# XMUDM/SPEX

Hardware: NVIDIA B200
Metric: lightgcn_propagation_gedges_per_s (higher is better)
Workload: dtype f32

## Files before the change

### include/spex_b200.h

```cpp
#ifndef SPEX_B200_H
#define SPEX_B200_H

#include <stdint.h>

#ifdef __cplusplus
extern "C" {
#endif

#define SPEX_ABI_VERSION 1

#define SPEX_E_BADARG   (-1)
#define SPEX_E_BADDIM   (-2)
#define SPEX_E_ALIGN    (-3)
#define SPEX_E_ARCH     (-4)
#define SPEX_E_TOOBIG   (-5)
#define SPEX_E_WORKSPACE (-6)

int spex_abi_version(void);
const char* spex_error_string(int code);
int spex_device_check(int* sm_count, int* cc_major, int* cc_minor);
int64_t spex_launch_count(void);

#define SPEX_PLAN_COL_HOTBIT 1
#define SPEX_PLAN_TWO_PASS 2
#define SPEX_PLAN_INTERLEAVE 4

typedef struct spex_long_plan {
  int32_t seg_len;
  int32_t n_long;
  int32_t n_seg;
  int32_t flags;
  const int32_t* long_rows;
  const int32_t* long_segptr;
  float* partial;
  const int64_t* seg_start;
  const int32_t* seg_count;
  const int32_t* row_seg;
  const int64_t* rowmid;
  float* hot_partial;
  int64_t n_split_rows;
  int64_t interleave_split;
} spex_long_plan;

int spex_spmm_csr_f32(const int64_t* rowptr, const int32_t* col, const float* val,
                      const float* X, int64_t n_rows, int32_t D,
                      float* Y, const float* addend, float addend_scale,
                      float* Z, float z_scale,
                      const spex_long_plan* plan, void* stream);

int spex_spmm_csr_rows_f32(const int64_t* rowptr, const int32_t* col, const float* val,
                           const float* X, int64_t n_rows, int32_t D,
                           const int32_t* rows, int64_t n_sel,
                           const int32_t* long_slots, int32_t n_long_sel,
                           const int32_t* seg_ids, int32_t n_seg_sel,
                           const uint8_t* x_nonzero,
                           float* Y, const float* addend, float addend_scale,
                           float* Z, float z_scale,
                           const spex_long_plan* plan, void* stream);

int spex_propagate_mean_f32(const int64_t* rowptr, const int32_t* col, const float* val,
                            const float* E0, int64_t N, int32_t D, int32_t K,
                            float* out, float* tmp0, float* tmp1,
                            const spex_long_plan* plan, void* stream);

int spex_propagate_mean_bwd_f32(const int64_t* rowptr, const int32_t* col, const float* valT,
                                const float* g, int64_t N, int32_t D, int32_t K,
                                float* dE0, float* tmp0, float* tmp1,
                                const spex_long_plan* plan, void* stream);

int spex_gather_f32(const float* src, const int64_t* idx, const float* scale, float divisor,
                    float* out, int64_t n, void* stream);

int spex_bce_fwd_f32(const float* U, const float* I, int32_t D,
                     const int64_t* users, const int64_t* items, const float* labels,
                     int64_t B, float* gamma, float* loss, float* dgamma, void* stream);

int spex_bce_bwd_f32(const float* U, const float* I, int32_t D,
                     const int64_t* users, const int64_t* items, const float* dgamma,
                     const float* grad_loss, int64_t B, float* gU, float* gI, void* stream);
int64_t spex_scatter_workspace_bytes(int64_t total_entries);
int spex_bce_bwd_ws_f32(const float* U, const float* I, int32_t D,
                        const int64_t* users, const int64_t* items, const float* dgamma,
                        const float* grad_loss, int64_t B, float* gU, float* gI,
                        void* work, int64_t work_bytes, void* stream);
int spex_clear_rows_f32(float* table, const int64_t* rows, int64_t n, int32_t D, void* stream);
int spex_gather_owned_rows_f32(const float* table_local, const int64_t* rows, int64_t n, int32_t D,
                               int64_t row_lo, int64_t row_hi, float* R, void* stream);
int spex_scatter_rows_f32(const int64_t* dst_rows, const int64_t* src_rows, const float* coef,
                          const float* gscalar, float cconst, int64_t B, const float* src, int32_t D,
                          float* out, int64_t row_lo, int64_t row_hi, void* work, int64_t work_bytes,
                          void* stream);

int spex_bpr_fwd_f32(const float* U, const float* I, const float* U0, const float* I0, int32_t D,
                     const int64_t* users, const int64_t* pos, const int64_t* neg, int64_t B,
// ... 126 lines not shown
```

### spex_b200/_capi.py

```python
from __future__ import annotations

import ctypes as C
import os

_HERE = os.path.dirname(os.path.abspath(__file__))
LIB_PATH = os.environ.get("SPEX_B200_LIB") or os.path.join(_HERE, "libspex_b200.so")

_p = C.c_void_p
_i32 = C.c_int32
_i64 = C.c_int64
_f = C.c_float


class LongPlan(C.Structure):

    _fields_ = [
        ("seg_len", _i32),
        ("n_long", _i32),
        ("n_seg", _i32),
        ("flags", _i32),
        ("long_rows", _p),
        ("long_segptr", _p),
        ("partial", _p),
        ("seg_start", _p),
        ("seg_count", _p),
        ("row_seg", _p),
        ("rowmid", _p),
        ("hot_partial", _p),
        ("n_split_rows", _i64),
        ("interleave_split", _i64),
    ]


_PLAN = C.POINTER(LongPlan)

SIGNATURES = {
    "spex_abi_version": (C.c_int, []),
    "spex_error_string": (C.c_char_p, [C.c_int]),
    "spex_device_check": (C.c_int, [C.POINTER(C.c_int)] * 3),
    "spex_launch_count": (_i64, []),
    "spex_spmm_csr_f32": (C.c_int, [_p, _p, _p, _p, _i64, _i32, _p, _p, _f, _p, _f, _PLAN, _p]),
    "spex_spmm_csr_rows_f32": (C.c_int, [_p, _p, _p, _p, _i64, _i32, _p, _i64, _p, _i32, _p, _i32, _p, _p, _p, _f, _p, _f,
                                         _PLAN, _p]),
    "spex_spmm_csr_rows_exchange_f32": (C.c_int, [_p, _p, _p, _p, _i64, _i32, _p, _i64, _p, _i32, _p, _i32, _p, _i64, _p,
                                                  _p, _i32, _p, _f, _p, _f, _PLAN, _p]),
    "spex_propagate_mean_f32": (C.c_int, [_p, _p, _p, _p, _i64, _i32, _i32, _p, _p, _p, _PLAN, _p]),
    "spex_propagate_mean_bwd_f32": (C.c_int, [_p, _p, _p, _p, _i64, _i32, _i32, _p, _p, _p, _PLAN, _p]),
    "spex_gather_f32": (C.c_int, [_p, _p, _p, _f, _p, _i64, _p]),
    "spex_bce_fwd_f32": (C.c_int, [_p, _p, _i32, _p, _p, _p, _i64, _p, _p, _p, _p]),
    "spex_bce_bwd_f32": (C.c_int, [_p, _p, _i32, _p, _p, _p, _p, _i64, _p, _p, _p]),
    "spex_scatter_workspace_bytes": (_i64, [_i64]),
    "spex_bce_bwd_ws_f32": (C.c_int, [_p, _p, _i32, _p, _p, _p, _p, _i64, _p, _p, _p, _i64, _p]),
    "spex_clear_rows_f32": (C.c_int, [_p, _p, _i64, _i32, _p]),
    "spex_gather_owned_rows_f32": (C.c_int, [_p, _p, _i64, _i32, _i64, _i64, _p, _p]),
    "spex_scatter_rows_f32": (C.c_int, [_p, _p, _p, _p, _f, _i64, _p, _i32, _p, _i64, _i64, _p, _i64, _p]),
    "spex_bpr_bwd_ws_f32": (C.c_int, [_p, _p, _p, _p, _i32, _p, _p, _p, _p, _p, _i64, _p, _p, _p, _p, _p, _i64, _p]),
    "spex_bpr_fwd_f32": (C.c_int, [_p, _p, _p, _p, _i32, _p, _p, _p, _i64, _p, _p, _p, _p]),
    "spex_bpr_bwd_f32": (C.c_int, [_p, _p, _p, _p, _i32, _p, _p, _p, _p, _p, _i64, _p, _p, _p, _p, _p]),
    "spex_adam_f32": (C.c_int, [_p, _p, _p, _p, _i64, _f, _f, _f, _f, _i32, _p]),
    "spex_sample_negatives": (C.c_int, [_p, _p, _i32, _i32, _p, _i64, _i32, C.c_uint64, _p, _p]),
    "spex_sample_bpr": (C.c_int, [_p, _p, _i32, _i32, _i64, _i64, C.c_uint64, _p, _p, _p, _p]),
    "spex_expert_gate_f32": (C.c_int, [_p, _p, _p, _i64, _i32, _p, _p]),
    "spex_expert_gate_bwd_f32": (C.c_int, [_p, _p, _p, _p, _i64, _i32, _p, _p, _p, _p, _p]),
    "spex_score_topk_f32": (C.c_int, [_p, _p, _i32, _p, _i64, _i64, _p, _p, _i32, _p, _p, _p]),
    "spex_rating_f32": (C.c_int, [_p, _p, _i32, _p, _i64, _i64, _i32, _p, _p]),
    "spex_pack_bf16": (C.c_int, [_p, _p, _i64, _i64, _i32, _p, _p]),
    "spex_score_topk_bf16": (C.c_int, [_p, _p, _i64, _i64, _i64, _i64, _p, _p, _p, _i32, _p, _p, _p]),
    "spex_pack_f16": (C.c_int, [_p, _p, _i64, _i64, _i32, _p, _p, _p]),
    "spex_score_topk_f16": (C.c_int, [_p, _p, _i32, _i64, _i64, _i64, _i64, _p, _p, _p, _p, _p, _i32, _p, _p, _p]),
    "spex_score_candidates_f32": (C.c_int, [_p, _p, _i32, _p, _p, _i64, _i32, _p, _p]),
    "spex_ngcf_epilogue_f32": (C.c_int, [_p, _p, _p, _p, _p, _p, _i64, _i32, _f, _p, _p, _i64, _p]),
    "spex_ngcf_layer_fwd_f32": (C.c_int, [_p, _p, _p, _p, _p, _p, _p, _i64, _i32, _f, _p, _p, _i64, _p]),
    "spex_ngcf_layer_bwd_f32": (C.c_int, [_p, _p, _p, _p, _p, _p, _p, _p, _p, _i64, _i64, _i32, _f, _p, _p, _p, _p,
                                          _p, _p, _p, _p]),
    "spex_ipc_alloc": (C.c_int, [_i64, C.POINTER(_p), _p]),
    "spex_ipc_open": (C.c_int, [_p, C.POINTER(_p)]),
    "spex_ipc_close": (C.c_int, [_p]),
    "spex_ipc_free": (C.c_int, [_p]),
    "spex_spmm_csr_f32_mcast": (C.c_int, [_p, _p, _p, _p, _i64, _i32, _i64, _p, _p, _f, _p, _f, _PLAN, _p]),
    "spex_mcast_rows_f32": (C.c_int, [_p, _i64, _i32, _i64, _p, _p]),
    "spex_mcast_rows_f32_ex": (C.c_int, [_p, _i64, _i32, _i64, _p, _i32, _p]),
    "spex_push_rows_f32_ex": (C.c_int, [_p, _i64, _i32, _i64, C.POINTER(_p), _i32, _i32, _p]),
    "spex_spmm_csr_f32_publish": (C.c_int, [_p, _p, _p, _p, _i64, _i32, _i64, _p, _f, _p, _f, _p, _p,
# ... 79 lines not shown
```

### spex_b200/csrc/spmm.cu

```cuda
#include "common.cuh"
#include <math.h>
#include <stdlib.h>

namespace spex {

int64_t g_launches = 0;

template <int D>
struct RowShape {
  static_assert(D == 32 || D == 64 || D == 128, "vector path supports D in {32,64,128}");
  static constexpr int LPR = D / 4;
  static constexpr int G = 32 / LPR;
};

template <int D, int U, int kMode, bool kFirst = false, bool kHot = false>
__device__ __forceinline__ float4 warp_row_accumulate(const int32_t* __restrict__ col,
                                                      const float* __restrict__ val,
                                                      const float* __restrict__ X, int64_t start,
                                                      int64_t end, int lane, int c0 = 0,
                                                      float v0 = 0.f) {
  constexpr int LPR = RowShape<D>::LPR, G = RowShape<D>::G;
  const int grp = lane / LPR, sub = lane % LPR;
  const float* Xs = X + sub * 4;
  float4 acc = f4_zero();
// ... 24 lines not shown
    const int n = (int)((end - base) < 32 ? (end - base) : 32);
#pragma unroll 1
    for (int j = 0; j < n; j += G * U) {
      float4 x[U];
      float vv[U];
#pragma unroll
      for (int u = 0; u < U; ++u) {
        const int idx = j + u * G + grp;
        const int cc = __shfl_sync(kFull, c, idx & 31);
        vv[u] = __shfl_sync(kFull, v, idx & 31);
        if (idx < n) {
          if (kHot)
            x[u] = ld_gather_f4_hint(Xs + (int64_t)(cc & 0x7fffffff) * D, cc < 0 ? pol_last : pol_first);
          else
            x[u] = ld_gather_f4(Xs + (int64_t)cc * D);
        } else {
          x[u] = f4_zero();
          vv[u] = 0.f;
        }
      }
#pragma unroll
      for (int u = 0; u < U; ++u) f4_fma(acc, vv[u], x[u]);
    }
  }
#pragma unroll
  for (int m = LPR; m < 32; m <<= 1) f4_add(acc, f4_shfl_xor(acc, m));
  return acc;
}

struct f8 {
  float4 a, b;
};
__device__ __forceinline__ f8 ld_gather_f8(const float* p) {
  f8 v;
  asm("ld.global.nc.L1::no_allocate.v8.f32 {%0,%1,%2,%3,%4,%5,%6,%7}, [%8];"
      : "=f"(v.a.x), "=f"(v.a.y), "=f"(v.a.z), "=f"(v.a.w), "=f"(v.b.x), "=f"(v.b.y), "=f"(v.b.z), "=f"(v.b.w)
      : "l"(p));
  return v;
}
__device__ __forceinline__ f8 ld_gather_f8_last(const float* p) {
  f8 v;
  asm("ld.global.nc.L1::no_allocate.L2::evict_last.v8.f32 {%0,%1,%2,%3,%4,%5,%6,%7}, [%8];"
      : "=f"(v.a.x), "=f"(v.a.y), "=f"(v.a.z), "=f"(v.a.w), "=f"(v.b.x), "=f"(v.b.y), "=f"(v.b.z), "=f"(v.b.w)
      : "l"(p));
  return v;
}
__device__ __forceinline__ f8 ld_gather_f8_first(const float* p) {
  f8 v;
  asm("ld.global.nc.L1::no_allocate.L2::evict_first.v8.f32 {%0,%1,%2,%3,%4,%5,%6,%7}, [%8];"
      : "=f"(v.a.x), "=f"(v.a.y), "=f"(v.a.z), "=f"(v.a.w), "=f"(v.b.x), "=f"(v.b.y), "=f"(v.b.z), "=f"(v.b.w)
      : "l"(p));
  return v;
}
template <int D, bool kHot>
__device__ __forceinline__ f8 gather_row8(const float* Xs, int cc) {
  const float* p;
  asm("mad.wide.u32 %0, %1, %2, %3;" : "=l"(p) : "r"(kHot ? (uint32_t)cc & 0x7fffffffu : (uint32_t)cc), "n"(D * 4), "l"(Xs));
  if (kHot) return cc < 0 ? ld_gather_f8_last(p) : ld_gather_f8_first(p);
  return ld_gather_f8(p);
}
__device__ __forceinline__ void f8_fma(f8& acc, float s, const f8& x) {
  f4_fma(acc.a, s, x.a);
  f4_fma(acc.b, s, x.b);
}

template <int D, int U, bool kHot>
__device__ __forceinline__ float4 warp_row_accumulate8(const int32_t* __restrict__ col,
                                                       const float* __restrict__ val,
                                                       const float* __restrict__ X, int64_t start,
                                                       int64_t end, int lane) {
  constexpr int LPR8 = D / 8;
  static_assert(LPR8 % U == 0, "U must divide the group's share of a batch");
  const int grp = lane / LPR8, sub = lane % LPR8;
  const float* Xs = X + sub * 8;
  f8 acc;
  acc.a = f4_zero();
  acc.b = f4_zero();
  int rem = (int)(end - start);
  const int32_t* cp = col + start + lane;
  const float* vp = val + start + lane;
  int c = 0;
  float v = 0.f;
  if (lane < rem) {
    c = ld_stream_s32(cp);
    v = ld_stream_f32(vp);
  }
  while (rem > 0) {
    int cn = 0;
    float vn = 0.f;
    if (lane + 32 < rem) {
      cn = ld_stream_s32(cp + 32);
      vn = ld_stream_f32(vp + 32);
    }
    if (rem >= 32) {
#pragma unroll
      for (int k0 = 0; k0 < LPR8; k0 += U) {
        f8 x[U];
        float vv[U];
#pragma unroll
        for (int u = 0; u < U; ++u) {
          const int cc = __shfl_sync(kFull, c, k0 + u, LPR8);
          vv[u] = __shfl_sync(kFull, v, k0 + u, LPR8);
          x[u] = gather_row8<D, kHot>(Xs, cc);
        }
#pragma unroll
        for (int u = 0; u < U; ++u) f8_fma(acc, vv[u], x[u]);
      }
    } else {
      const int ng = rem - grp * LPR8;
      const int nmax = rem < LPR8 ? rem : LPR8;
#pragma unroll 1
      for (int k0 = 0; k0 < nmax; k0 += U) {
        f8 x[U];
        float vv[U];
#pragma unroll
        for (int u = 0; u < U; ++u) {
          const int cc = __shfl_sync(kFull, c, k0 + u, LPR8);
          vv[u] = __shfl_sync(kFull, v, k0 + u, LPR8);
          if (k0 + u < ng) {
            x[u] = gather_row8<D, kHot>(Xs, cc);
          } else {
            x[u].a = f4_zero();
            x[u].b = f4_zero();
            vv[u] = 0.f;
          }
        }
#pragma unroll
        for (int u = 0; u < U; ++u) f8_fma(acc, vv[u], x[u]);
      }
    }
    c = cn;
    v = vn;
    cp += 32;
    vp += 32;
    rem -= 32;
  }
#pragma unroll
  for (int m = LPR8; m < 32; m <<= 1) {
    f4_add(acc.a, f4_shfl_xor(acc.a, m));
    f4_add(acc.b, f4_shfl_xor(acc.b, m));
  }
  const int src = (lane >> 1) & (LPR8 - 1);
  float4 lo, hi;
  lo.x = __shfl_sync(kFull, acc.a.x, src);
  lo.y = __shfl_sync(kFull, acc.a.y, src);
  lo.z = __shfl_sync(kFull, acc.a.z, src);
  lo.w = __shfl_sync(kFull, acc.a.w, src);
  hi.x = __shfl_sync(kFull, acc.b.x, src);
  hi.y = __shfl_sync(kFull, acc.b.y, src);
  hi.z = __shfl_sync(kFull, acc.b.z, src);
  hi.w = __shfl_sync(kFull, acc.b.w, src);
  return (lane & 1) ? hi : lo;
}

#ifndef SPEX_V8_U
#define SPEX_V8_U 4
#endif
#ifndef SPEX_MASK_U
#define SPEX_MASK_U 2
#endif
#ifndef SPEX_V8_MINB
#define SPEX_V8_MINB 32
#endif
template <int D, bool kHot>
__device__ __forceinline__ float4 warp_row_accumulate8_masked(const int32_t* __restrict__ col,
                                                              const float* __restrict__ val,
                                                              const float* __restrict__ X,
                                                              const uint8_t* __restrict__ nz, int64_t start,
                                                              int64_t end, int lane) {
  constexpr int LPR8 = D / 8;
  constexpr int U = SPEX_MASK_U;
  const int grp = lane / LPR8, sub = lane % LPR8;
  const float* Xs = X + sub * 8;
  f8 acc;
  acc.a = f4_zero();
  acc.b = f4_zero();
  int rem = (int)(end - start);
  const int32_t* cp = col + start + lane;
  const float* vp = val + start + lane;
  constexpr uint32_t kIdMask = kHot ? 0x7fffffffu : 0xffffffffu;
  int c = 0, cn = 0;
  float v = 0.f, vn = 0.f;
  bool on = false;
  if (lane < rem) {
    c = ld_stream_s32(cp);
    v = ld_stream_f32(vp);
  }
  if (lane + 32 < rem) {
    cn = ld_stream_s32(cp + 32);
    vn = ld_stream_f32(vp + 32);
  }
  if (lane < rem) on = nz[(uint32_t)c & kIdMask] != 0;
  while (rem > 0) {
    int c2 = 0;
// ... 185 lines not shown
                     const int32_t* __restrict__ long_rows,
                     const int32_t* __restrict__ long_segptr, int32_t n_long, int32_t n_seg,
                     int32_t seg_len, float* __restrict__ partial, const int32_t* __restrict__ seg_sel,
                     const uint8_t* __restrict__ nz) {
  constexpr int LPR = RowShape<D>::LPR;
  const int lane = threadIdx.x & 31;
  int seg = blockIdx.x * kRowsPerCta + (threadIdx.x >> 5);
  if (seg >= n_seg) return;
  if (seg_sel) seg = seg_sel[seg];
  int lo = 0, hi = n_long;
  while (hi - lo > 1) {
    const int mid = (lo + hi) >> 1;
    if (long_segptr[mid] <= seg) lo = mid; else hi = mid;
  }
  const int64_t row = long_rows[lo];
  const int k = seg - long_segptr[lo];
  const int64_t rs = rowptr[row], re = rowptr[row + 1];
  const int64_t start = rs + (int64_t)k * seg_len;
  const int64_t end = (start + seg_len < re) ? start + seg_len : re;
  const float4 acc = row_sum<D, U, kHot, kV8, kMask>(col, val, X, start, end, lane, nz);
  if (lane < LPR) *reinterpret_cast<float4*>(partial + (int64_t)seg * D + lane * 4) = acc;
}

template <int D, int U>
__global__ void __launch_bounds__(kRowsPerCta * 32)
spmm_long_fix_kernel(const int32_t* __restrict__ long_rows,
                     const int32_t* __restrict__ long_segptr, int32_t n_long,
                     const float* __restrict__ partial, Epilogue ep, const int32_t* __restrict__ slot_sel) {
  const int lane = threadIdx.x & 31;
  int r = blockIdx.x * kRowsPerCta + (threadIdx.x >> 5);
  if (r >= n_long) return;
  if (slot_sel) r = slot_sel[r];
  const float4 acc = warp_row_accumulate<D, U, 1>(nullptr, nullptr, partial, long_segptr[r],
                                                  long_segptr[r + 1], lane);
  row_epilogue<D>(ep, acc, (int64_t)long_rows[r], lane);
}

template <int D, int U, bool kHot, bool kV8, bool kMask>
__global__ void __launch_bounds__(kRowsPerCta * 32, SPEX_V8_MINB / kRowsPerCta)
spmm_seg_list_kernel(const int32_t* __restrict__ col, const float* __restrict__ val,
                     const float* __restrict__ X, const int64_t* __restrict__ seg_start,
                     const int32_t* __restrict__ seg_count, int32_t n_seg, float* __restrict__ partial,
                     const int32_t* __restrict__ seg_sel, const uint8_t* __restrict__ nz) {
  constexpr int LPR = RowShape<D>::LPR;
  const int lane = threadIdx.x & 31;
  int seg = blockIdx.x * kRowsPerCta + (threadIdx.x >> 5);
  if (seg >= n_seg) return;
  if (seg_sel) seg = seg_sel[seg];
  const int64_t start = seg_start[seg];
  const float4 acc = row_sum<D, U, kHot, kV8, kMask>(col, val, X, start, start + seg_count[seg], lane, nz);
  if (lane < LPR) *reinterpret_cast<float4*>(partial + (int64_t)seg * D + lane * 4) = acc;
}

template <int D, int U>
__global__ void __launch_bounds__(kRowsPerCta * 32)
spmm_long_fix_list_kernel(const int32_t* __restrict__ long_rows,
                          const int32_t* __restrict__ long_segptr, const int32_t* __restrict__ row_seg,
                          int32_t n_long, const float* __restrict__ partial, Epilogue ep,
                          const int32_t* __restrict__ slot_sel) {
  const int lane = threadIdx.x & 31;
  int r = blockIdx.x * kRowsPerCta + (threadIdx.x >> 5);
  if (r >= n_long) return;
  if (slot_sel) r = slot_sel[r];
  const float4 acc = warp_row_accumulate<D, U, 2>(row_seg, nullptr, partial, long_segptr[r],
                                                  long_segptr[r + 1], lane);
  row_epilogue<D>(ep, acc, (int64_t)long_rows[r], lane);
}

template <int NV>
__global__ void __launch_bounds__(kRowsPerCta * 32)
spmm_rows_generic_kernel(const int64_t* __restrict__ rowptr, const int32_t* __restrict__ col,
                         const float* __restrict__ val, const float* __restrict__ X,
                         int64_t n_rows, int32_t D, Epilogue ep) {
  const int lane = threadIdx.x & 31;
  const int64_t row = (int64_t)blockIdx.x * kRowsPerCta + (threadIdx.x >> 5);
  if (row >= n_rows) return;
  const int64_t start = rowptr[row], end = rowptr[row + 1];
  float4 acc[NV];
#pragma unroll
  for (int v = 0; v < NV; ++v) acc[v] = f4_zero();
  for (int64_t base = start; base < end; base += 32) {
    const int64_t e = base + lane;
    int c = 0;
    float w = 0.f;
    if (e < end) {
      c = ld_stream_s32(col + e);
      w = ld_stream_f32(val + e);
    }
    const int n = (int)((end - base) < 32 ? (end - base) : 32);
    for (int j = 0; j < n; ++j) {
      const int cc = __shfl_sync(kFull, c, j);
      const float ww = __shfl_sync(kFull, w, j);
#pragma unroll
      for (int v = 0; v < NV; ++v) {
        const int d = (lane + 32 * v) * 4;
        if (d < D) f4_fma(acc[v], ww, ld_gather_f4(X + (int64_t)cc * D + d));
      }
    }
  }
#pragma unroll
  for (int v = 0; v < NV; ++v) {
    const int d = (lane + 32 * v) * 4;
    if (d < D) {
      const int64_t off = row * D + d;
      if (ep.Y) *reinterpret_cast<float4*>(ep.Y + off) = acc[v];
      if (ep.mcast) {
        st_multimem_f4(ep.mcast + (row + ep.peer_row_offset) * D + d, acc[v]);
      } else {
        for (int p = 0; p < ep.n_peers; ++p)
          *reinterpret_cast<float4*>(ep.peer[p] + (row + ep.peer_row_offset) * D + d) = acc[v];
      }
      if (ep.Z) {
        float4 a = f4_zero();
        if (ep.addend) a = ld_f4(ep.addend + off);
        float4 z;
        z.x = (a.x * ep.addend_scale + acc[v].x) * ep.z_scale;
        z.y = (a.y * ep.addend_scale + acc[v].y) * ep.z_scale;
        z.z = (a.z * ep.addend_scale + acc[v].z) * ep.z_scale;
        z.w = (a.w * ep.addend_scale + acc[v].w) * ep.z_scale;
        *reinterpret_cast<float4*>(ep.Z + off) = z;
      }
    }
  }
}

static bool g_rows_only = false;

struct RowSubset {
  const int32_t* rows;
  int64_t n_rows;
  const int32_t* long_slots;
  int32_t n_long;
  const int32_t* seg_ids;
  int32_t n_seg;
};

template <int D, int U, bool kHot, bool kV8, bool kMask>
static int launch_vec_h(const int64_t* rowptr, const int32_t* col, const float* val, const float* X,
                        int64_t n_rows, const Epilogue& ep, const spex_long_plan* plan,
                        cudaStream_t st, const RowSubset* sub, const uint8_t* nz) {
  const bool rows_only = g_rows_only;
  const bool has_long = plan && plan->n_long > 0;
  const int64_t n_work = sub ? sub->n_rows : n_rows;
  const int64_t grid = (n_work + kRowsPerCta - 1) / kRowsPerCta;
  if (grid > 0x7fffffffLL) return SPEX_E_TOOBIG;
  const int64_t split = (!sub && plan && (plan->flags & SPEX_PLAN_INTERLEAVE) && plan->interleave_split > 0 &&
                         plan->interleave_split < n_rows)
                            ? plan->interleave_split
                            : 0;
  const int32_t* row_sel = sub ? sub->rows : nullptr;
  if (!sub && !kMask && kHot && plan && (plan->flags & SPEX_PLAN_TWO_PASS) && plan->rowmid && plan->hot_partial) {
    const int64_t nA = plan->n_split_rows < n_rows ? plan->n_split_rows : n_rows;
    Epilogue epA{};
    epA.Y = plan->hot_partial;
    const int64_t gridA = (nA + kRowsPerCta - 1) / kRowsPerCta;
    if (gridA > 0) {
      spmm_rows_kernel<D, U, kHot, kV8, false><<<(unsigned)gridA, kRowsPerCta * 32, 0, st>>>(
          rowptr, col, val, X, nA, has_long ? plan->seg_len : 0, epA, plan->rowmid, 1, 0, nullptr, nullptr);
      count_launch();
    }
    Epilogue epB = ep;
    epB.partial_in = plan->hot_partial;
    epB.n_partial = nA;
    spmm_rows_kernel<D, U, kHot, kV8, false><<<(unsigned)grid, kRowsPerCta * 32, 0, st>>>(
        rowptr, col, val, X, n_rows, has_long ? plan->seg_len : 0, epB, plan->rowmid, 2, split, nullptr, nullptr);
    count_launch();
  } else if (grid > 0) {
    spmm_rows_kernel<D, U, kHot, kV8, kMask><<<(unsigned)grid, kRowsPerCta * 32, 0, st>>>(
        rowptr, col, val, X, n_work, has_long ? plan->seg_len : 0, ep, nullptr, 0, split, row_sel, nz);
    count_launch();
  }
  if (rows_only) return check_last();
  if (has_long) {
    const int32_t n_seg = sub ? sub->n_seg : plan->n_seg;
    const int32_t n_long = sub ? sub->n_long : plan->n_long;
    const int32_t* seg_sel = sub ? sub->seg_ids : nullptr;
    const int32_t* slot_sel = sub ? sub->long_slots : nullptr;
    if (n_long == 0) return check_last();
    const int gs = (n_seg + kRowsPerCta - 1) / kRowsPerCta;
    const int gf = (n_long + kRowsPerCta - 1) / kRowsPerCta;
    if (plan->seg_start) {
      spmm_seg_list_kernel<D, U, kHot, kV8, kMask><<<gs, kRowsPerCta * 32, 0, st>>>(
          col, val, X, plan->seg_start, plan->seg_count, n_seg, plan->partial, seg_sel, nz);
      spmm_long_fix_list_kernel<D, U><<<gf, kRowsPerCta * 32, 0, st>>>(
          plan->long_rows, plan->long_segptr, plan->row_seg, n_long, plan->partial, ep, slot_sel);
    } else {
      spmm_long_seg_kernel<D, U, kHot, kV8, kMask><<<gs, kRowsPerCta * 32, 0, st>>>(
          rowptr, col, val, X, plan->long_rows, plan->long_segptr, plan->n_long, n_seg,
          plan->seg_len, plan->partial, seg_sel, nz);
      spmm_long_fix_kernel<D, U><<<gf, kRowsPerCta * 32, 0, st>>>(
          plan->long_rows, plan->long_segptr, n_long, plan->partial, ep, slot_sel);
    }
    count_launch(2);
  }
  return check_last();
}

template <int D, int U>
static int launch_vec(const int64_t* rowptr, const int32_t* col, const float* val, const float* X,
                      int64_t n_rows, const Epilogue& ep, const spex_long_plan* plan,
                      cudaStream_t st, const RowSubset* sub, const uint8_t* nz) {
  static const bool force128 = [] {
    const char* e = getenv("SPEX_SPMM_LDG128");
    return e && e[0] == '1';
  }();
  const bool v8 = !force128 && (reinterpret_cast<uintptr_t>(X) & 31u) == 0;
  const bool hot = plan && (plan->flags & SPEX_PLAN_COL_HOTBIT);
  if (nz && v8) {
    if (hot) return launch_vec_h<D, U, true, true, true>(rowptr, col, val, X, n_rows, ep, plan, st, sub, nz);
    return launch_vec_h<D, U, false, true, true>(rowptr, col, val, X, n_rows, ep, plan, st, sub, nz);
  }
  if (hot) {
    if (v8) return launch_vec_h<D, U, true, true, false>(rowptr, col, val, X, n_rows, ep, plan, st, sub, nullptr);
    return launch_vec_h<D, U, true, false, false>(rowptr, col, val, X, n_rows, ep, plan, st, sub, nullptr);
  }
  if (v8) return launch_vec_h<D, U, false, true, false>(rowptr, col, val, X, n_rows, ep, plan, st, sub, nullptr);
  return launch_vec_h<D, U, false, false, false>(rowptr, col, val, X, n_rows, ep, plan, st, sub, nullptr);
}

int spmm_launch(const int64_t* rowptr, const int32_t* col, const float* val, const float* X,
                int64_t n_rows, int32_t D, const Epilogue& ep, const spex_long_plan* plan,
                cudaStream_t st, const RowSubset* sub = nullptr, const uint8_t* nz = nullptr) {
  SPEX_RETURN_IF(!rowptr || !X || n_rows < 0, SPEX_E_BADARG);
  SPEX_RETURN_IF(n_rows > 0 && (!col || !val), SPEX_E_BADARG);
  SPEX_RETURN_IF(D <= 0 || (D & 3) || D > 512, SPEX_E_BADDIM);
  SPEX_RETURN_IF(!aligned16(X) || !aligned16(ep.Y) || !aligned16(ep.Z) || !aligned16(ep.addend),
                 SPEX_E_ALIGN);
  if (plan && plan->n_long > 0) {
    SPEX_RETURN_IF(plan->seg_len < 32 || !plan->long_rows || !plan->long_segptr ||
                       !plan->partial || plan->n_seg < plan->n_long,
                   SPEX_E_BADARG);
    SPEX_RETURN_IF(plan->seg_start && (!plan->seg_count || !plan->row_seg), SPEX_E_BADARG);
    SPEX_RETURN_IF(!aligned16(plan->partial), SPEX_E_ALIGN);
  }
  if (n_rows == 0) return 0;
  switch (D) {
    case 32: return launch_vec<32, 4>(rowptr, col, val, X, n_rows, ep, plan, st, sub, nz);
    case 64: return launch_vec<64, SPEX_U64>(rowptr, col, val, X, n_rows, ep, plan, st, sub, nz);
    case 128: return launch_vec<128, 8>(rowptr, col, val, X, n_rows, ep, plan, st, sub, nz);
    default: break;
  }
  SPEX_RETURN_IF(sub != nullptr, SPEX_E_BADDIM);
  SPEX_RETURN_IF(plan && (plan->flags & SPEX_PLAN_COL_HOTBIT), SPEX_E_BADDIM);
  SPEX_RETURN_IF(ep.partial_in != nullptr || ep.pub_src != nullptr || ep.adam_p != nullptr, SPEX_E_BADDIM);
  const int64_t grid = (n_rows + kRowsPerCta - 1) / kRowsPerCta;
  if (grid > 0x7fffffffLL) return SPEX_E_TOOBIG;
  const int nv = (D + 127) / 128;
  switch (nv) {
    case 1: spmm_rows_generic_kernel<1><<<(unsigned)grid, kRowsPerCta * 32, 0, st>>>(rowptr, col, val, X, n_rows, D, ep); break;
    case 2: spmm_rows_generic_kernel<2><<<(unsigned)grid, kRowsPerCta * 32, 0, st>>>(rowptr, col, val, X, n_rows, D, ep); break;
    case 3: spmm_rows_generic_kernel<3><<<(unsigned)grid, kRowsPerCta * 32, 0, st>>>(rowptr, col, val, X, n_rows, D, ep); break;
    default: spmm_rows_generic_kernel<4><<<(unsigned)grid, kRowsPerCta * 32, 0, st>>>(rowptr, col, val, X, n_rows, D, ep); break;
  }
  count_launch();
  return check_last();
}

__global__ void copy_f4_kernel(const float4* __restrict__ src, float4* __restrict__ dst, int64_t n4) {
  int64_t i = (int64_t)blockIdx.x * blockDim.x + threadIdx.x;
  const int64_t stride = (int64_t)gridDim.x * blockDim.x;
  for (; i < n4; i += stride) dst[i] = src[i];
}

struct PeerTables {
  float* peer[8];
  int n_peers;
};
__global__ void __launch_bounds__(256)
push_rows_kernel(const float4* __restrict__ src, int64_t n4, int64_t dst_off4, PeerTables pt) {
  int64_t i = (int64_t)blockIdx.x * blockDim.x + threadIdx.x;
  const int64_t stride = (int64_t)gridDim.x * blockDim.x;
  const int rot = blockIdx.x % pt.n_peers;
  for (; i < n4; i += stride) {
    const float4 v = ld_stream_f4(reinterpret_cast<const float*>(src + i));
#pragma unroll
    for (int p = 0; p < 8; ++p) {
      if (p < pt.n_peers) {
        int q = p + rot;
        if (q >= pt.n_peers) q -= pt.n_peers;
        reinterpret_cast<float4*>(pt.peer[q])[dst_off4 + i] = v;
      }
    }
  }
}

// ... 322 lines not shown
```

### spex_b200/ops.py

```python
from __future__ import annotations

import ctypes as C
from typing import Optional

import numpy as np
import torch

from . import _capi
from ._capi import LongPlan, call, ptr, stream_ptr
from .graph import CSRGraph, DEFAULT_SEG_LEN, plan_long_rows


class _Workspaces:

    def __init__(self):
        self.enabled = False
        self.buf = {}
        self.dirty = {}

    def get(self, name, shape, device, zero=False):
        key = (name, tuple(shape), str(device))
        t = self.buf.get(key) if self.enabled else None
        if t is None:
            t = (torch.zeros if zero else torch.empty)(*shape, dtype=torch.float32, device=device)
# ... 69 lines not shown
        self.n_rows = rowptr.numel() - 1
        self.n_cols = int(n_cols)
        self.nnz = col.numel()
        self.tpos = tpos
        self.row_offset = int(row_offset)
        self.symmetric = symmetric
        self.device = val.device
        self.seg_len = int(seg_len)
        self._plan_struct = None
        self._plan_D = 0
        self._plan_tensors = None
        self.interleave_split = 0
        self.rowmid = None
        self.n_split_rows = 0
        self.col_hot = False
        if col_hot:
            self.col_hot = True
        self._build_plan(D_hint)

    @classmethod
    def from_host(cls, g: CSRGraph, device, seg_len: int = DEFAULT_SEG_LEN, D_hint: int = 64):
        dev = torch.device(device)
        rowptr = torch.from_numpy(np.ascontiguousarray(g.rowptr)).to(dev)
        col = torch.from_numpy(np.ascontiguousarray(g.col)).to(dev)
        val = torch.from_numpy(np.ascontiguousarray(g.val)).to(dev)
        tpos = None if g.tpos is None else torch.from_numpy(np.ascontiguousarray(g.tpos)).to(dev)
        return cls(rowptr, col, val, g.n_cols, tpos, seg_len, g.row_offset, D_hint=D_hint)

    @classmethod
    def from_sparse_coo(cls, A: torch.Tensor, device, seg_len: int = DEFAULT_SEG_LEN):
        A = A.coalesce()
        idx = A.indices()
        n_rows, n_cols = A.shape
        dev = torch.device(device)
        rows = idx[0].to(dev)
        counts = torch.bincount(rows, minlength=n_rows)
        rowptr = torch.zeros(n_rows + 1, dtype=torch.int64, device=dev)
        torch.cumsum(counts, 0, out=rowptr[1:])
        col = idx[1].to(dev).to(torch.int32)
        val = A.values().to(dev).to(torch.float32)
        return cls(rowptr, col, val, n_cols, None, seg_len)

    L2_WINDOW_BYTES = 16 << 20
    MIN_CB_COLS = 1024
    HUB_EDGES_PER_BLOCK = 16

    def _build_plan(self, D: int):
        dev = self.device
        deg = self.rowptr[1:] - self.rowptr[:-1]
        long_rows = torch.nonzero(deg > self.seg_len).flatten()
        self.n_long = int(long_rows.numel())
        self.long_rows = long_rows.to(torch.int32)
        self.seg_start = self.seg_count = self.row_seg = None
        self._plan_D = 0
        if self.n_long == 0:
            self.long_segptr = torch.zeros(1, dtype=torch.int32, device=dev)
            self.n_seg = 0
            return
        table_bytes = self.n_cols * D * 4
        if table_bytes <= 4 * self.L2_WINDOW_BYTES:
            nseg = (deg[long_rows] + self.seg_len - 1) // self.seg_len
            segptr = torch.zeros(self.n_long + 1, dtype=torch.int64, device=dev)
            torch.cumsum(nseg, 0, out=segptr[1:])
            self.long_segptr = segptr.to(torch.int32)
            self.n_seg = int(segptr[-1].item())
            return
        import os as _os
        win = int(_os.environ.get("SPEX_L2_WINDOW_MB", 0)) << 20 or self.L2_WINDOW_BYTES
        epb = int(_os.environ.get("SPEX_HUB_EPB", 0)) or self.HUB_EDGES_PER_BLOCK
        cb_cols = max(win // (D * 4), self.MIN_CB_COLS)
        n_cb = (self.n_cols + cb_cols - 1) // cb_cols
        ldeg = deg[long_rows]
        is_hub = ldeg >= epb * n_cb
        hub_slots = torch.nonzero(is_hub).flatten()
        mid_slots = torch.nonzero(~is_hub).flatten()
        parts_start, parts_cnt, parts_row = [], [], []
        if hub_slots.numel():
            hrows = long_rows[hub_slots]
            nh = hrows.numel()
            lo = self.rowptr[hrows].unsqueeze(1).expand(nh, n_cb + 1).clone()
            hi = self.rowptr[hrows + 1].unsqueeze(1).expand(nh, n_cb + 1).clone()
            target = (torch.arange(n_cb + 1, device=dev, dtype=torch.int64) * cb_cols).unsqueeze(0)
            steps = int(ldeg.max().item()).bit_length() + 1
            last = self.nnz - 1
            for _ in range(steps):
                mid = (lo + hi) >> 1
                go = ((self.col[mid.clamp(max=last)] & 0x7FFFFFFF).to(torch.int64) < target) & (lo < hi)
                lo = torch.where(go, mid + 1, lo)
                hi = torch.where(go, hi, mid)
            pos = lo
            del lo, hi, mid, go
            cs = pos[:, :-1].t().reshape(-1)
            cc = (pos[:, 1:] - pos[:, :-1]).t().reshape(-1)
            cr = hub_slots.repeat(n_cb)
            keep = cc > 0
            parts_start.append(cs[keep]); parts_cnt.append(cc[keep]); parts_row.append(cr[keep])
        if mid_slots.numel():
            mrows = long_rows[mid_slots]
            parts_start.append(self.rowptr[mrows]); parts_cnt.append(deg[mrows]); parts_row.append(mid_slots)
        cell_start = torch.cat(parts_start)
        cell_cnt = torch.cat(parts_cnt)
        cell_row = torch.cat(parts_row)
        pieces = (cell_cnt + self.seg_len - 1) // self.seg_len
        seg_cell = torch.repeat_interleave(torch.arange(cell_cnt.numel(), device=dev), pieces)
        first = torch.cumsum(pieces, 0) - pieces
        piece_idx = torch.arange(seg_cell.numel(), device=dev) - first[seg_cell]
        seg_start = cell_start[seg_cell] + piece_idx * self.seg_len
        seg_end = torch.minimum(seg_start + self.seg_len, (cell_start + cell_cnt)[seg_cell])
        seg_row = cell_row[seg_cell]
        self.n_seg = int(seg_start.numel())
        self.n_hub = int(hub_slots.numel())
        if self.n_seg >= 2 ** 31:
            raise ValueError("too many long-row segments")
        order = torch.sort(seg_row * (self.nnz + 1) + seg_start, stable=True).indices
        counts = torch.bincount(seg_row, minlength=self.n_long)
        segptr = torch.zeros(self.n_long + 1, dtype=torch.int64, device=dev)
        torch.cumsum(counts, 0, out=segptr[1:])
        self.long_segptr = segptr.to(torch.int32)
        self.seg_start = seg_start.contiguous()
        self.seg_count = (seg_end - seg_start).to(torch.int32).contiguous()
        self.row_seg = order.to(torch.int32).contiguous()

    HOT_L2_BYTES = 48 << 20

    def mark_hot_columns(self, D: int, col_degree: Optional[torch.Tensor] = None,
                         budget_bytes: Optional[int] = None) -> int:
        if self.col_hot:
            return -1
        import os as _os
        budget = budget_bytes if budget_bytes is not None else (
            int(_os.environ.get("SPEX_HOT_L2_MB", 0)) << 20 or self.HOT_L2_BYTES)
        n_hot = min(budget // (D * 4), self.n_cols)
        if self.n_cols * D * 4 <= 2 * budget or n_hot <= 0 or D not in (32, 64, 128):
            return 0
        if col_degree is None:
            if self.n_rows != self.n_cols:
                raise ValueError("column degrees are needed for a non-square graph")
            col_degree = self.rowptr[1:] - self.rowptr[:-1]
        thr = torch.topk(col_degree, n_hot).values[-1]
        hot = col_degree >= torch.clamp(thr, min=2)
        if int(hot.sum()) > 2 * n_hot:
            return 0
        chunk = 1 << 28
        int_min = -(2 ** 31)
        for s0 in range(0, self.nnz, chunk):
            c = self.col[s0: s0 + chunk]
            c.bitwise_or_(hot[c.long()].to(torch.int32) * int_min)
        self.col_hot = True
        self._plan_D = 0
        return int(hot.sum())

    def split_hot_cold(self, n_split_rows: Optional[int] = None, chunk_edges: int = 1 << 27) -> int:
        if not self.col_hot:
            return 0
        if self.tpos is not None:
            raise ValueError("split_hot_cold would invalidate the transpose map (edge dropout graphs)")
        n_split = self.n_rows if n_split_rows is None else min(int(n_split_rows), self.n_rows)
        dev = self.device
        rowptr = self.rowptr
        rowmid = rowptr[:-1].clone()
        total_hot = 0
        rp_host = rowptr[: n_split + 1].cpu()
        a = 0
        while a < n_split:
# ... 8 lines not shown
                rid = torch.repeat_interleave(torch.arange(b - a, device=dev), d)
                h = (c < 0) & (d <= self.seg_len)[rid]
                cs0 = torch.zeros(eb - ea + 1, dtype=torch.int64, device=dev)
                cs0[1:] = torch.cumsum(h, 0, dtype=torch.int64)
                hot_before = cs0[:-1] - cs0[lrp[:-1]][rid]
                hot_cnt = cs0[lrp[1:]] - cs0[lrp[:-1]]
                pos = torch.arange(eb - ea, device=dev) - lrp[:-1][rid]
                newpos = lrp[:-1][rid] + torch.where(h, hot_before, hot_cnt[rid] + (pos - hot_before))
                cn, vn = torch.empty_like(c), torch.empty_like(v)
                cn[newpos] = c
                vn[newpos] = v
                c.copy_(cn)
                v.copy_(vn)
                rowmid[a:b] += hot_cnt
                total_hot += int(hot_cnt.sum())
                del rid, h, cs0, hot_before, hot_cnt, pos, newpos, cn, vn
            a = b
        self.rowmid = rowmid
        self.n_split_rows = n_split
        self._plan_D = 0
        return total_hot

    def set_row_classes(self, split: int):
        self.interleave_split = int(split)
        self._plan_D = 0

    def clean_col(self) -> torch.Tensor:
        return (self.col & 0x7FFFFFFF) if self.col_hot else self.col

    def plan(self, D: int):
        inter = 0 < self.interleave_split < self.n_rows
        if self.n_long == 0 and not self.col_hot and not inter:
            return None
        flags = 1 if self.col_hot else 0
        two = self.col_hot and self.rowmid is not None
        if two:
            flags |= 2
        if inter:
            flags |= 4
        if self._plan_D != D:
            hot_partial = (torch.empty(self.n_split_rows * D, dtype=torch.float32, device=self.device)
                           if two else None)
            tail = (self.rowmid.data_ptr() if two else None, hot_partial.data_ptr() if two else None,
                    self.n_split_rows if two else 0, self.interleave_split if inter else 0)
            if self.n_long == 0:
                st = LongPlan(self.seg_len, 0, 0, flags, None, None, None, None, None, None, *tail)
                self._plan_tensors = (None, hot_partial)
            else:
                partial = torch.empty(self.n_seg * D, dtype=torch.float32, device=self.device)
                st = LongPlan(self.seg_len, self.n_long, self.n_seg, flags, self.long_rows.data_ptr(),
                              self.long_segptr.data_ptr(), partial.data_ptr(),
                              self.seg_start.data_ptr() if self.seg_start is not None else None,
                              self.seg_count.data_ptr() if self.seg_count is not None else None,
                              self.row_seg.data_ptr() if self.row_seg is not None else None, *tail)
                self._plan_tensors = (partial, hot_partial)
            self._plan_struct = st
            self._plan_D = D
        return C.byref(self._plan_struct)

    def _edge_positions(self, rows: torch.Tensor):
        a = self.rowptr[rows]
        cnt = self.rowptr[rows + 1] - a
        total = int(cnt.sum().item())
        first = torch.cumsum(cnt, 0) - cnt
        pos = torch.repeat_interleave(a - first, cnt, output_size=total) + torch.arange(total, device=self.device)
        return pos, total

    def degree_sum(self, rows: torch.Tensor) -> int:
        return int((self.rowptr[rows + 1] - self.rowptr[rows]).sum().item())

    def neighbors(self, rows: torch.Tensor) -> torch.Tensor:
        pos, total = self._edge_positions(rows)
        if total == 0:
            return torch.empty(0, dtype=torch.int64, device=self.device)
        c = self.col[pos]
        if self.col_hot:
            c = c & 0x7FFFFFFF
        return torch.unique(c.to(torch.int64))

    def row_subset(self, rows: torch.Tensor):
        rows = rows.to(torch.int64)
        r32 = rows.to(torch.int32).contiguous()
        if self.n_long == 0:
            return r32, None, None
        deg = self.rowptr[rows + 1] - self.rowptr[rows]
        lr = rows[deg > self.seg_len]
        if lr.numel() == 0:
            return r32, None, None
        slots = torch.searchsorted(self.long_rows.to(torch.int64), lr)
        segptr = self.long_segptr.to(torch.int64)
        a = segptr[slots]
        cnt = segptr[slots + 1] - a
        total = int(cnt.sum().item())
        first = torch.cumsum(cnt, 0) - cnt
        pos = torch.repeat_interleave(a - first, cnt, output_size=total) + torch.arange(total, device=self.device)
        seg_ids = self.row_seg[pos] if self.row_seg is not None else pos.to(torch.int32)
        return r32, slots.to(torch.int32).contiguous(), seg_ids.to(torch.int32).contiguous()

    def with_values(self, val: torch.Tensor, symmetric: bool) -> "DeviceGraph":
        g = object.__new__(DeviceGraph)
        g.__dict__.update(self.__dict__)
        g.val = val
        g.symmetric = symmetric
        return g

    def transposed_values(self, val: torch.Tensor) -> torch.Tensor:
        if self.tpos is None:
# ... 535 lines not shown
```

Measured before the change: 37.10.

## Process long-row segments in per-warp runs with hub/mid cache policy split

Adds a segment-runs kernel in which one warp handles a run of consecutive long-row segments (8 for hub segments, 2 for mid segments). It prefetches the next segment's column and value indices across segment boundaries and uses different gather cache hints for hub versus mid segments. The plan records how many segments belong to hub rows so the kernel can split them. The aim is to cut per-segment launch and latency overhead and to improve L2 reuse for hub gathers. The cost is 32-thread CTAs, which may hurt occupancy or scheduling, and a new ABI field in the plan struct.

```diff
diff --git a/include/spex_b200.h b/include/spex_b200.h
--- a/include/spex_b200.h
+++ b/include/spex_b200.h
@@ -40,6 +40,7 @@
   float* hot_partial;
   int64_t n_split_rows;
   int64_t interleave_split;
+  int32_t n_hub_seg;
 } spex_long_plan;
 
 int spex_spmm_csr_f32(const int64_t* rowptr, const int32_t* col, const float* val,
diff --git a/spex_b200/_capi.py b/spex_b200/_capi.py
--- a/spex_b200/_capi.py
+++ b/spex_b200/_capi.py
@@ -29,6 +29,7 @@
         ("hot_partial", _p),
         ("n_split_rows", _i64),
         ("interleave_split", _i64),
+        ("n_hub_seg", _i32),
     ]
 
 
diff --git a/spex_b200/csrc/spmm.cu b/spex_b200/csrc/spmm.cu
--- a/spex_b200/csrc/spmm.cu
+++ b/spex_b200/csrc/spmm.cu
@@ -100,16 +100,68 @@
       : "l"(p));
   return v;
 }
-template <int D, bool kHot>
+template <int D, bool kHot, bool kCold = kHot>
 __device__ __forceinline__ f8 gather_row8(const float* Xs, int cc) {
   const float* p;
   asm("mad.wide.u32 %0, %1, %2, %3;" : "=l"(p) : "r"(kHot ? (uint32_t)cc & 0x7fffffffu : (uint32_t)cc), "n"(D * 4), "l"(Xs));
-  if (kHot) return cc < 0 ? ld_gather_f8_last(p) : ld_gather_f8_first(p);
-  return ld_gather_f8(p);
+  if (kHot) return cc < 0 ? ld_gather_f8_last(p) : (kCold ? ld_gather_f8_first(p) : ld_gather_f8(p));
+  return kCold ? ld_gather_f8_first(p) : ld_gather_f8(p);
 }
 __device__ __forceinline__ void f8_fma(f8& acc, float s, const f8& x) {
   f4_fma(acc.a, s, x.a);
   f4_fma(acc.b, s, x.b);
+}
+
+template <int D, int U, bool kHot, bool kCold = kHot>
+__device__ __forceinline__ void batch_accumulate8(f8& acc, const float* Xs, int c, float v, int rem, int grp) {
+  constexpr int LPR8 = D / 8;
+  static_assert(LPR8 % U == 0, "U must divide the group's share of a batch");
+  if (rem >= 32) {
+#pragma unroll
+    for (int k0 = 0; k0 < LPR8; k0 += U) {
+      f8 x[U];
+      float vv[U];
+#pragma unroll
+      for (int u = 0; u < U; ++u) {
+        const int cc = __shfl_sync(kFull, c, k0 + u, LPR8);
+        vv[u] = __shfl_sync(kFull, v, k0 + u, LPR8);
+        x[u] = gather_row8<D, kHot, kCold>(Xs, cc);
+      }
+#pragma unroll
+      for (int u = 0; u < U; ++u) f8_fma(acc, vv[u], x[u]);
+    }
+  } else {
+    const int ng = rem - grp * LPR8;
+    const int nmax = rem < LPR8 ? rem : LPR8;
+#pragma unroll 1
+    for (int k0 = 0; k0 < nmax; k0 += U) {
+      f8 x[U];
+      float vv[U];
+#pragma unroll
+      for (int u = 0; u < U; ++u) {
+        const int cc = __shfl_sync(kFull, c, k0 + u, LPR8);
+        vv[u] = __shfl_sync(kFull, v, k0 + u, LPR8);
+        if (k0 + u < ng) {
+          x[u] = gather_row8<D, kHot, kCold>(Xs, cc);
+        } else {
+          x[u].a = f4_zero();
+          x[u].b = f4_zero();
+          vv[u] = 0.f;
+        }
+      }
+#pragma unroll
+      for (int u = 0; u < U; ++u) f8_fma(acc, vv[u], x[u]);
+    }
+  }
+}
+
+template <int D>
+__device__ __forceinline__ void groups_reduce8(f8& acc) {
+#pragma unroll
+  for (int m = D / 8; m < 32; m <<= 1) {
+    f4_add(acc.a, f4_shfl_xor(acc.a, m));
+    f4_add(acc.b, f4_shfl_xor(acc.b, m));
+  }
 }
 
 template <int D, int U, bool kHot>
@@ -118,7 +170,6 @@
                                                        const float* __restrict__ X, int64_t start,
                                                        int64_t end, int lane) {
   constexpr int LPR8 = D / 8;
-  static_assert(LPR8 % U == 0, "U must divide the group's share of a batch");
   const int grp = lane / LPR8, sub = lane % LPR8;
   const float* Xs = X + sub * 8;
   f8 acc;
@@ -140,54 +191,14 @@
       cn = ld_stream_s32(cp + 32);
       vn = ld_stream_f32(vp + 32);
     }
-    if (rem >= 32) {
-#pragma unroll
-      for (int k0 = 0; k0 < LPR8; k0 += U) {
-        f8 x[U];
-        float vv[U];
-#pragma unroll
-        for (int u = 0; u < U; ++u) {
-          const int cc = __shfl_sync(kFull, c, k0 + u, LPR8);
-          vv[u] = __shfl_sync(kFull, v, k0 + u, LPR8);
-          x[u] = gather_row8<D, kHot>(Xs, cc);
-        }
-#pragma unroll
-        for (int u = 0; u < U; ++u) f8_fma(acc, vv[u], x[u]);
-      }
-    } else {
-      const int ng = rem - grp * LPR8;
-      const int nmax = rem < LPR8 ? rem : LPR8;
-#pragma unroll 1
-      for (int k0 = 0; k0 < nmax; k0 += U) {
-        f8 x[U];
-        float vv[U];
-#pragma unroll
-        for (int u = 0; u < U; ++u) {
-          const int cc = __shfl_sync(kFull, c, k0 + u, LPR8);
-          vv[u] = __shfl_sync(kFull, v, k0 + u, LPR8);
-          if (k0 + u < ng) {
-            x[u] = gather_row8<D, kHot>(Xs, cc);
-          } else {
-            x[u].a = f4_zero();
-            x[u].b = f4_zero();
-            vv[u] = 0.f;
-          }
-        }
-#pragma unroll
-        for (int u = 0; u < U; ++u) f8_fma(acc, vv[u], x[u]);
-      }
-    }
+    batch_accumulate8<D, U, kHot>(acc, Xs, c, v, rem, grp);
     c = cn;
     v = vn;
     cp += 32;
     vp += 32;
     rem -= 32;
   }
-#pragma unroll
-  for (int m = LPR8; m < 32; m <<= 1) {
-    f4_add(acc.a, f4_shfl_xor(acc.a, m));
-    f4_add(acc.b, f4_shfl_xor(acc.b, m));
-  }
+  groups_reduce8<D>(acc);
   const int src = (lane >> 1) & (LPR8 - 1);
   float4 lo, hi;
   lo.x = __shfl_sync(kFull, acc.a.x, src);
@@ -479,6 +490,95 @@
   if (lane < LPR) *reinterpret_cast<float4*>(partial + (int64_t)seg * D + lane * 4) = acc;
 }
 
+#ifndef SPEX_SEG_HUB_RUN
+#define SPEX_SEG_HUB_RUN 8
+#endif
+#ifndef SPEX_SEG_MID_RUN
+#define SPEX_SEG_MID_RUN 2
+#endif
+constexpr int kHubRun = SPEX_SEG_HUB_RUN, kMidRun = SPEX_SEG_MID_RUN;
+static_assert(kHubRun <= 32 && kMidRun <= 32, "a run's segment extents are held one per lane");
+
+template <int D, bool kHot, bool kCold>
+__device__ __forceinline__ void seg_run8(const int32_t* __restrict__ col, const float* __restrict__ val,
+                                         const float* __restrict__ X, const int64_t* __restrict__ seg_start,
+                                         const int32_t* __restrict__ seg_count, int first, int n,
+                                         float* __restrict__ partial, int lane) {
+  constexpr int LPR8 = D / 8, U = D >= 64 ? SPEX_V8_U : D / 8;
+  const int grp = lane / LPR8, sub = lane % LPR8;
+  const float* Xs = X + sub * 8;
+  int64_t my_start = 0;
+  int my_cnt = 0;
+  if (lane < n) {
+    my_start = seg_start[first + lane];
+    my_cnt = seg_count[first + lane];
+  }
+  int64_t start = __shfl_sync(kFull, my_start, 0);
+  int rem = __shfl_sync(kFull, my_cnt, 0);
+  int c = 0;
+  float v = 0.f;
+  if (lane < rem) {
+    c = ld_stream_s32(col + start + lane);
+    v = ld_stream_f32(val + start + lane);
+  }
+#pragma unroll 1
+  for (int k = 0; k < n; ++k) {
+    const int64_t nstart = __shfl_sync(kFull, my_start, (k + 1) & 31);
+    const int ncnt = k + 1 < n ? __shfl_sync(kFull, my_cnt, (k + 1) & 31) : 0;
+    f8 acc;
+    acc.a = f4_zero();
+    acc.b = f4_zero();
+    int64_t e = start + lane;
+#pragma unroll 1
+    while (rem > 0) {
+      int cn = 0;
+      float vn = 0.f;
+      if (rem > 32) {
+        if (lane + 32 < rem) {
+          cn = ld_stream_s32(col + e + 32);
+          vn = ld_stream_f32(val + e + 32);
+        }
+      } else if (lane < ncnt) {
+        cn = ld_stream_s32(col + nstart + lane);
+        vn = ld_stream_f32(val + nstart + lane);
+      }
+      batch_accumulate8<D, U, kHot, kCold>(acc, Xs, c, v, rem, grp);
+      c = cn;
+      v = vn;
+      e += 32;
+      rem -= 32;
+    }
+    groups_reduce8<D>(acc);
+    if (lane < LPR8) {
+      float* p = partial + (int64_t)(first + k) * D + lane * 8;
+      st_stream_f4(p, acc.a);
+      st_stream_f4(p + 4, acc.b);
+    }
+    start = nstart;
+    rem = ncnt;
+  }
+}
+
+template <int D, bool kHot>
+__global__ void __launch_bounds__(32, SPEX_V8_MINB)
+spmm_seg_runs_kernel(const int32_t* __restrict__ col, const float* __restrict__ val, const float* __restrict__ X,
+                     const int64_t* __restrict__ seg_start, const int32_t* __restrict__ seg_count, int32_t n_seg,
+                     int32_t n_hub_seg, float* __restrict__ partial) {
+  const int lane = threadIdx.x;
+  const int hub_warps = (n_hub_seg + kHubRun - 1) / kHubRun;
+  const int w = blockIdx.x;
+  if (w < hub_warps) {
+    const int first = w * kHubRun;
+    const int n = min(kHubRun, n_hub_seg - first);
+    seg_run8<D, kHot, false>(col, val, X, seg_start, seg_count, first, n, partial, lane);
+  } else {
+    const int first = n_hub_seg + (w - hub_warps) * kMidRun;
+    if (first >= n_seg) return;
+    const int n = min(kMidRun, n_seg - first);
+    seg_run8<D, kHot, kHot>(col, val, X, seg_start, seg_count, first, n, partial, lane);
+  }
+}
+
 template <int D, int U>
 __global__ void __launch_bounds__(kRowsPerCta * 32)
 spmm_long_fix_list_kernel(const int32_t* __restrict__ long_rows,
@@ -552,6 +652,11 @@
 }
 
 static bool g_rows_only = false;
+
+static bool seg_legacy() {
+  const char* e = getenv("SPEX_SPMM_SEG_LEGACY");
+  return e && e[0] == '1';
+}
 
 struct RowSubset {
   const int32_t* rows;
@@ -607,8 +712,15 @@
     const int gs = (n_seg + kRowsPerCta - 1) / kRowsPerCta;
     const int gf = (n_long + kRowsPerCta - 1) / kRowsPerCta;
     if (plan->seg_start) {
-      spmm_seg_list_kernel<D, U, kHot, kV8, kMask><<<gs, kRowsPerCta * 32, 0, st>>>(
-          col, val, X, plan->seg_start, plan->seg_count, n_seg, plan->partial, seg_sel, nz);
+      if (kV8 && !kMask && !sub && !seg_legacy()) {
+        const int n_mid = n_seg - plan->n_hub_seg;
+        const int gr = (plan->n_hub_seg + kHubRun - 1) / kHubRun + (n_mid + kMidRun - 1) / kMidRun;
+        spmm_seg_runs_kernel<D, kHot><<<gr, 32, 0, st>>>(col, val, X, plan->seg_start, plan->seg_count, n_seg,
+                                                         plan->n_hub_seg, plan->partial);
+      } else {
+        spmm_seg_list_kernel<D, U, kHot, kV8, kMask><<<gs, kRowsPerCta * 32, 0, st>>>(
+            col, val, X, plan->seg_start, plan->seg_count, n_seg, plan->partial, seg_sel, nz);
+      }
       spmm_long_fix_list_kernel<D, U><<<gf, kRowsPerCta * 32, 0, st>>>(
           plan->long_rows, plan->long_segptr, plan->row_seg, n_long, plan->partial, ep, slot_sel);
     } else {
@@ -658,6 +770,7 @@
                        !plan->partial || plan->n_seg < plan->n_long,
                    SPEX_E_BADARG);
     SPEX_RETURN_IF(plan->seg_start && (!plan->seg_count || !plan->row_seg), SPEX_E_BADARG);
+    SPEX_RETURN_IF(plan->n_hub_seg < 0 || plan->n_hub_seg > plan->n_seg, SPEX_E_BADARG);
     SPEX_RETURN_IF(!aligned16(plan->partial), SPEX_E_ALIGN);
   }
   if (n_rows == 0) return 0;
diff --git a/spex_b200/ops.py b/spex_b200/ops.py
--- a/spex_b200/ops.py
+++ b/spex_b200/ops.py
@@ -145,6 +145,7 @@
         self.n_long = int(long_rows.numel())
         self.long_rows = long_rows.to(torch.int32)
         self.seg_start = self.seg_count = self.row_seg = None
+        self.n_hub_seg = 0
         self._plan_D = 0
         if self.n_long == 0:
             self.long_segptr = torch.zeros(1, dtype=torch.int32, device=dev)
@@ -168,6 +169,7 @@
         hub_slots = torch.nonzero(is_hub).flatten()
         mid_slots = torch.nonzero(~is_hub).flatten()
         parts_start, parts_cnt, parts_row = [], [], []
+        n_hub_cells = 0
         if hub_slots.numel():
             hrows = long_rows[hub_slots]
             nh = hrows.numel()
@@ -188,6 +190,7 @@
             cr = hub_slots.repeat(n_cb)
             keep = cc > 0
             parts_start.append(cs[keep]); parts_cnt.append(cc[keep]); parts_row.append(cr[keep])
+            n_hub_cells = int(parts_cnt[0].numel())
         if mid_slots.numel():
             mrows = long_rows[mid_slots]
             parts_start.append(self.rowptr[mrows]); parts_cnt.append(deg[mrows]); parts_row.append(mid_slots)
@@ -203,6 +206,7 @@
         seg_row = cell_row[seg_cell]
         self.n_seg = int(seg_start.numel())
         self.n_hub = int(hub_slots.numel())
+        self.n_hub_seg = int(pieces[:n_hub_cells].sum())
         if self.n_seg >= 2 ** 31:
             raise ValueError("too many long-row segments")
         order = torch.sort(seg_row * (self.nnz + 1) + seg_start, stable=True).indices
@@ -317,7 +321,8 @@
                               self.long_segptr.data_ptr(), partial.data_ptr(),
                               self.seg_start.data_ptr() if self.seg_start is not None else None,
                               self.seg_count.data_ptr() if self.seg_count is not None else None,
-                              self.row_seg.data_ptr() if self.row_seg is not None else None, *tail)
+                              self.row_seg.data_ptr() if self.row_seg is not None else None, *tail,
+                              self.n_hub_seg)
                 self._plan_tensors = (partial, hot_partial)
             self._plan_struct = st
             self._plan_D = D
```

After: 40.06 (median of 6 runs). 8.0% higher.
